# OPTML-Group/Unlearn-Saliency

Measured on AMD Instinct MI355X. Metric: unlearn_steps_per_sec (ResNet-18/CIFAR-10 10%-forget, RL + SalUn mask, batch 256/GPU), higher is better.
Workload: dtype f32

## Files before the change

### include/salun.h

```cpp
#ifndef SALUN_H
#define SALUN_H

#include <stddef.h>
#include <stdint.h>

#ifdef __cplusplus
extern "C" {
#endif

#define SALUN_OK 0
#define SALUN_EINVAL (-22)
#define SALUN_ENOSPC (-28)
#define SALUN_EIO (-5)

#define SALUN_MAX_THRESHOLDS 16

typedef void *salun_stream_t;

int salun_version(void);
const char *salun_strerror(int code);
const char *salun_arch(void);
int salun_clock_probe(unsigned long long *out , int samples, int spins, salun_stream_t stream);

int salun_saliency_accumulate(float *acc , const float *g ,
// ... 82 lines not shown
                               salun_stream_t stream);
int salun_conv2d_backward_data_add(const float *dy , const float *w , const float *addend ,
                                   float *dx , int N, int C, int H, int W, int K, int R, int stride, int pad,
                                   int P, int Q, salun_stream_t stream);
size_t salun_channel_sum_workspace_bytes(int N, int K);
int salun_channel_sum(const float *dy , float *out , int N, int K, int HW, int accumulate,
                      void *ws , size_t ws_bytes, salun_stream_t stream);
size_t salun_conv2d_wgrad_workspace_bytes(int N, int C, int K, int R, int P, int Q);
int salun_conv2d_backward_weight(const float *x , const float *dy , float *dw , int N, int C,
                                 int H, int W, int K, int R, int stride, int pad, int P, int Q, int accumulate,
                                 void *ws , size_t ws_bytes, salun_stream_t stream);
#define SALUN_WGRAD_SHARED 1u
int salun_conv2d_backward_weight_ex(const float *x , const float *dy , float *dw , int N, int C,
                                    int H, int W, int K, int R, int stride, int pad, int P, int Q, int accumulate,
                                    unsigned flags, void *ws , size_t ws_bytes, salun_stream_t stream);
#define SALUN_ROUTE_FORWARD 0
#define SALUN_ROUTE_BACKWARD_DATA 1
#define SALUN_ROUTE_BACKWARD_WEIGHT 2
#define SALUN_ROUTE_EPI 2u
#define SALUN_ROUTE_W_UNALIGNED 4u
#define SALUN_ROUTE_OUT_UNALIGNED 8u
#define SALUN_ROUTE_IN_UNALIGNED 16u
int salun_conv2d_route(int direction, int N, int C, int H, int W, int K, int R, int stride, int pad, int P, int Q,
                       unsigned flags, size_t ws_bytes, char *buf, size_t buflen, int *nsplit );

size_t salun_conv3x3_pack_bytes(int K, int C, int dgrad);
#define SALUN_PACK_MAX_JOBS 32
typedef struct {
  const float *w;
  float *img_fwd;
  float *img_dgrad;
  int32_t K, C;
} salun_pack_job_t;
int salun_conv3x3_pack_weights(const salun_pack_job_t *jobs , int njobs, salun_stream_t stream);
int salun_conv3x3_packed(const float *x , const float *img , const float *bias ,
                         const float *nbias , const float *addend , float *y ,
                         int N, int Cred, int H, int W, int Kout, int cfg, salun_stream_t stream);
// ... 300 lines not shown
```

### unlearn_saliency_amd/_lib.py

```python
from __future__ import annotations

import ctypes
import os
import subprocess

_HERE = os.path.dirname(os.path.abspath(__file__))
LIB_PATH = os.environ.get("SALUN_LIB") or os.path.join(_HERE, "libsalun.so")
CSRC_DIR = os.path.join(_HERE, "csrc")

SALUN_OK = 0
SALUN_EINVAL = -22
SALUN_ENOSPC = -28
SALUN_EIO = -5
SALUN_MAX_THRESHOLDS = 16
SALUN_TOPK_FORCE_FULL_SCAN = 1
SALUN_TOPK_VALUES_ONLY = 2
SALUN_WGRAD_SHARED = 1

c_void_p, c_int, c_int64, c_uint64 = ctypes.c_void_p, ctypes.c_int, ctypes.c_int64, ctypes.c_uint64
c_double, c_size_t = ctypes.c_double, ctypes.c_size_t

class GemmSeg(ctypes.Structure):
    _fields_ = [("A", c_void_p), ("B", c_void_p), ("K", ctypes.c_int32), ("a_i", ctypes.c_int32),
                ("a_k", ctypes.c_int32), ("b_j", ctypes.c_int32), ("b_k", ctypes.c_int32)]
# ... 75 lines not shown
    "salun_conv2d_forward": (c_int, [c_void_p, c_void_p, c_void_p, c_void_p] + [c_int] * 10 + [c_void_p]),
    "salun_conv2d_forward_fused": (c_int, [c_void_p] * 6 + [c_int] * 10 + [c_void_p, c_size_t, c_void_p]),
    "salun_conv2d_data_workspace_bytes": (c_size_t, [c_int] * 6),
    "salun_conv2d_backward_data_ws": (c_int, [c_void_p] * 4 + [c_int] * 10 + [c_void_p, c_size_t, c_void_p]),
    "salun_conv2d_backward_data": (c_int, [c_void_p, c_void_p, c_void_p] + [c_int] * 10 + [c_void_p]),
    "salun_channel_sum_workspace_bytes": (c_size_t, [c_int] * 2),
    "salun_channel_sum": (c_int, [c_void_p, c_void_p] + [c_int] * 4 + [c_void_p, c_size_t, c_void_p]),
    "salun_conv2d_wgrad_workspace_bytes": (c_size_t, [c_int] * 6),
    "salun_conv3x3_pack_bytes": (c_size_t, [c_int] * 3),
    "salun_conv3x3_pack_weights": (c_int, [c_void_p, c_int, c_void_p]),
    "salun_conv3x3_packed": (c_int, [c_void_p] * 6 + [c_int] * 6 + [c_void_p]),
    "salun_conv2d_backward_weight": (c_int, [c_void_p, c_void_p, c_void_p] + [c_int] * 11 + [c_void_p, c_size_t,
                                                                                          c_void_p]),
    "salun_conv2d_backward_weight_ex": (c_int, [c_void_p, c_void_p, c_void_p] + [c_int] * 11 + [ctypes.c_uint, c_void_p,
                                                                                                 c_size_t, c_void_p]),
    "salun_conv2d_route": (c_int, [c_int] * 11 + [ctypes.c_uint, c_size_t, ctypes.c_char_p, c_size_t,
                                   ctypes.POINTER(c_int)]),
    "salun_conv2d_bf16_supported": (c_int, [c_int] * 5),
    "salun_conv2d_bf16_pack_weights": (c_int, [c_void_p, c_void_p, c_int, c_int, c_int, c_void_p]),
    "salun_bf16_pack_weights_batch": (c_int, [c_void_p, c_int, c_void_p]),
    "salun_conv2d_bf16_data_workspace_bytes": (c_size_t, [c_int] * 8),
    "salun_conv2d_bf16_forward": (c_int, [c_void_p] * 6 + [c_int] * 8 + [c_void_p, c_size_t, c_void_p]),
    "salun_conv2d_bf16_backward_data": (c_int, [c_void_p] * 4 + [c_int] * 8 + [c_void_p, c_size_t, c_void_p]),
    "salun_conv2d_bf16_wgrad_workspace_bytes": (c_size_t, [c_int] * 8),
    "salun_conv2d_bf16_backward_weight": (c_int, [c_void_p] * 4 + [c_int] * 9 + [c_void_p, c_size_t, c_void_p]),
    "salun_colsum_bf16_workspace_bytes": (c_size_t, [c_int]),
    "salun_colsum_bf16": (c_int, [c_void_p, c_void_p, c_void_p, c_int64, c_int, c_int, c_int, c_void_p, c_size_t, c_void_p]),
    "salun_conv2d_bf16_backward_weight_ex": (c_int, [c_void_p] * 5 + [c_int] * 9 + [c_void_p, c_size_t, c_void_p]),
    "salun_conv2d_bf16_route": (c_int, [c_int] * 9 + [ctypes.c_uint, c_size_t, ctypes.c_char_p, c_size_t,
                                        ctypes.POINTER(c_int)]),
# ... 138 lines not shown
```

### unlearn_saliency_amd/csrc/salun_conv.hip

```cpp
#include "salun_common.h"
#include "salun_conv_plan.h"
#include <mutex>
#include <type_traits>
#include <unordered_set>

int salun_ring_wgrad_launch(const float *x, const float *dy, float *part, int N, int C, int H, int W, int K, int nsplit,
                            int nchunks, hipStream_t st);

namespace {

typedef float f32x16 __attribute__((ext_vector_type(16)));

struct PatchPos {
  int goff;
  int loff;
  int valid;
};

__device__ __forceinline__ void tile_origin(int tile, int NI, int TP, int tiles_per_img, int &n0, int &p0) {
  if (NI > 1) { n0 = tile * NI; p0 = 0; }
  else { n0 = tile / tiles_per_img; p0 = (tile - n0 * tiles_per_img) * TP; }
}

struct LanePix {
// ... 784 lines not shown
    }
  }
  float *out = part + (size_t)split * K * C * RS;
  const int c = c0 + ct * 32 + lo;
  if (c < C) {
#pragma unroll
    for (int t = 0; t < RS; ++t)
#pragma unroll
      for (int v = 0; v < 16; ++v) {
        const int k = k0 + kt * 32 + (v & 3) + 8 * (v >> 2) + 4 * hi;
        if (k < K) out[((size_t)t * K + k) * C + c] = acc[t][v];
      }
  }
}

template <int STRIDE, int NIT>
__global__ __launch_bounds__(256) void conv_wgrad_v(const float *__restrict__ x, const float *__restrict__ dy,
                                                    float *__restrict__ part, int N, int C, int H, int W, int K, int P,
                                                    int Q, int NI, int TP, int IH_t, int IW_t, int logQ, int nchunks) {
  constexpr int R = 3, RS = 9, PAD = 1;
  constexpr int PIXC = (STRIDE == 1) ? 64 : 32;
  constexpr int DROW = PIXC + 1;
  constexpr int NSTEP = PIXC / 2;
  constexpr int HALF = NSTEP / 2;
  constexpr int DN4 = 64 * PIXC / 4 / 256;
  constexpr int LOGPIX4 = (PIXC == 64) ? 4 : 3;
  constexpr int NLD = NIT + DN4;
  constexpr int LPS = (NLD + HALF - 1) / HALF;
  constexpr int NST = 4 * (NIT + DN4);
  constexpr int SPS = (NST + HALF - 1) / HALF;
  static_assert(LPS <= RS && SPS <= RS, "one staging instruction per MFMA slot at most");
  extern __shared__ __attribute__((aligned(16))) float lds[];
  const int PSZ = NI * IH_t * IW_t;
  const int ch_stride = PSZ | 1;
  const int BUF = 64 * ch_stride + 64 * DROW + 256;

  const int tid = threadIdx.x, lane = tid & 63, wave = tid >> 6;
  const int lo = lane & 31, hi = lane >> 5;
  const int kt = wave & 1, ct = wave >> 1;
  const int k0 = blockIdx.x * 64, c0 = blockIdx.y * 64;
  const int split = blockIdx.z, nsplit = gridDim.z;
  const int tiles_per_img = (NI > 1) ? 1 : P / TP;
  const int planeHW = H * W, PQ = P * Q;
  const int logTP = __builtin_ctz(TP);
  const int W4 = W >> 2;
  const int F4C = NI * IH_t * W4;

  f32x16 acc[RS];
#pragma unroll
  for (int t = 0; t < RS; ++t)
#pragma unroll
    for (int v = 0; v < 16; ++v) acc[t][v] = 0.f;

  int it_lds[NIT];
  int it_g[NIT];
  int it_ih[NIT], it_ni[NIT];
#pragma unroll
  for (int k = 0; k < NIT; ++k) {
    const int e = tid + k * 256;
    const int c = e / F4C, r = e - c * F4C;
    const int ni = r / (IH_t * W4), r2 = r - ni * (IH_t * W4);
    const int ih = r2 / W4, g4 = r2 - ih * W4;
    it_lds[k] = c * ch_stride + (ni * IH_t + ih) * IW_t + PAD + 4 * g4;
    it_g[k] = (ni * C + c) * planeHW + (ih - PAD) * W + 4 * g4;
    it_ih[k] = ih;
    it_ni[k] = ni;
  }
  float4 xreg[NIT];
  float4 dreg[DN4];
  const float *xbase = x;
  unsigned xoff[NIT], xmask[NIT];
  const float *dbase = dy;
  unsigned doff[DN4], dmask[DN4];
  int d_kk[DN4], d_ni[DN4], d_in[DN4];
#pragma unroll
  for (int i = 0; i < DN4; ++i) {
    const int e4 = tid + i * 256;
    const int kk = e4 >> LOGPIX4, m = (e4 & (PIXC / 4 - 1)) * 4;
    const int q = m & (Q - 1), pr = m >> logQ;
    d_kk[i] = kk;
    d_ni[i] = pr >> logTP;
    d_in[i] = (pr & (TP - 1)) * Q + q;
  }
  auto aim = [&](int chunk) {
    int n0, p0;
    if (NI > 1) { n0 = chunk * NI; p0 = 0; }
    else { n0 = chunk / tiles_per_img; p0 = (chunk - n0 * tiles_per_img) * TP; }
    xbase = x + ((size_t)n0 * C + c0) * planeHW;
    const int h0 = p0 * STRIDE;
#pragma unroll
    for (int k = 0; k < NIT; ++k) {
      const int h = h0 - PAD + it_ih[k];
      const bool ok = (n0 + it_ni[k]) < N && h >= 0 && h < H;
      xoff[k] = ok ? (unsigned)(it_g[k] + h0 * W) : 0u;
      xmask[k] = ok ? 0xffffffffu : 0u;
    }
    dbase = dy + ((size_t)n0 * K + k0) * PQ + (size_t)p0 * Q;
#pragma unroll
    for (int i = 0; i < DN4; ++i) {
      const bool okd = (n0 + d_ni[i]) < N && (k0 + d_kk[i]) < K;
      doff[i] = okd ? (unsigned)((d_ni[i] * K + d_kk[i]) * PQ + d_in[i]) : 0u;
      dmask[i] = okd ? 0xffffffffu : 0u;
    }
  };
  auto load_item = [&](int li) {
    if (li < NIT) xreg[li] = *reinterpret_cast<const float4 *>(xbase + xoff[li]);
    else dreg[li - NIT] = *reinterpret_cast<const float4 *>(dbase + doff[li - NIT]);
  };
  auto comp_of = [](const float4 &v, int comp) { return comp == 0 ? v.x : comp == 1 ? v.y : comp == 2 ? v.z : v.w; };
  auto store_item = [&](float *buf, int si) {
    if (si < 4 * NIT) {
      const int k = si >> 2, comp = si & 3;
      buf[it_lds[k] + comp] = __uint_as_float(__float_as_uint(comp_of(xreg[k], comp)) & xmask[k]);
    } else {
      const int sd = si - 4 * NIT, i = sd >> 2, comp = sd & 3;
      const int e4 = tid + i * 256;
      const int kk = e4 >> LOGPIX4, m = (e4 & (PIXC / 4 - 1)) * 4 + comp;
      (buf + 64 * ch_stride)[kk * DROW + m] = __uint_as_float(__float_as_uint(comp_of(dreg[i], comp)) & dmask[i]);
    }
  };

  for (int i = tid; i < 2 * BUF; i += 256) lds[i] = 0.f;
  __syncthreads();

  if (split < nchunks) {
    aim(split);
#pragma unroll
    for (int li = 0; li < NLD; ++li) load_item(li);
#pragma unroll
    for (int si = 0; si < NST; ++si) store_item(lds, si);
    __syncthreads();

    int cur = 0;
    for (int chunk = split; chunk < nchunks; chunk += nsplit) {
      const float *xp = lds + cur * BUF;
      const float *dl = xp + 64 * ch_stride;
      float *buf_n = lds + (cur ^ 1) * BUF;
      aim(chunk + nsplit < nchunks ? chunk + nsplit : chunk);
      const float *arow = dl + (kt * 32 + lo) * DROW + hi;
      const float *brow = xp + (ct * 32 + lo) * ch_stride + hi * STRIDE;
      auto pair_off = [&](int j) {
        const int q0 = j & (Q - 1), pr = j >> logQ;
        const int ni = pr >> logTP, pl = pr & (TP - 1);
        return (ni * IH_t + pl * STRIDE) * IW_t + q0 * STRIDE;
      };
      float a_cur, b_cur[RS], a_nxt = 0.f, b_nxt[RS];
      {
        const float *bp = brow + pair_off(0);
        a_cur = arow[0];
#pragma unroll
        for (int t = 0; t < RS; ++t) b_cur[t] = bp[(t / R) * IW_t + (t % R)];
      }
#pragma unroll
      for (int st = 0; st < NSTEP; ++st) {
        const float *bp = brow + ((st + 1 < NSTEP) ? pair_off(2 * st + 2) : 0);
#pragma unroll
        for (int t = 0; t < RS; ++t) {
          acc[t] = __builtin_amdgcn_mfma_f32_32x32x2f32(a_cur, b_cur[t], acc[t], 0, 0, 0);
          __builtin_amdgcn_sched_barrier(0);
          if (st + 1 < NSTEP) {
            if (t == 0) a_nxt = arow[2 * st + 2];
            b_nxt[t] = bp[(t / R) * IW_t + (t % R)];
          }
          if (st < HALF) {
            if (t < LPS && st * LPS + t < NLD) load_item(st * LPS + t);
          } else {
            if (t < SPS && (st - HALF) * SPS + t < NST) store_item(buf_n, (st - HALF) * SPS + t);
          }
          __builtin_amdgcn_sched_barrier(0);
        }
        a_cur = a_nxt;
#pragma unroll
        for (int t = 0; t < RS; ++t) b_cur[t] = b_nxt[t];
      }
      __syncthreads();
      cur ^= 1;
    }
  }
  float *out = part + (size_t)split * K * C * RS;
  const int c = c0 + ct * 32 + lo;
#pragma unroll
  for (int t = 0; t < RS; ++t)
#pragma unroll
    for (int v = 0; v < 16; ++v) {
      const int k = k0 + kt * 32 + (v & 3) + 8 * (v >> 2) + 4 * hi;
      if (k < K) out[((size_t)t * K + k) * C + c] = acc[t][v];
    }
}

template <int STRIDE>
__global__ __launch_bounds__(256) void conv_wgrad_1x1(const float *__restrict__ x, const float *__restrict__ dy,
                                                      float *__restrict__ part, int N, int C, int H, int W, int K,
                                                      int P, int Q, int nchunks) {
  constexpr int PIXC = 64, DROW = PIXC + 1, NSTEP = PIXC / 2, HALF = NSTEP / 2;
  constexpr int NA = 128 * PIXC / 4 / 256;
  constexpr int NB = NA;
  constexpr int NLD = NA + NB * STRIDE;
  constexpr int LPS = (NLD + HALF - 1) / HALF;
  constexpr int NST = 4 * (NA + NB);
  constexpr int SPS = (NST + HALF - 1) / HALF;
  static_assert(LPS <= 4 && SPS <= 4, "one staging instruction per MFMA slot");
  constexpr int BUF = 2 * 128 * DROW;
// ... 540 lines not shown
  int N, C, H, W, K, P, Q, pad;
};

template <int STRIDE>
void launch_one_wgrad_1x1(const WgradPlan &p, const WgradArgs &a, hipStream_t st) {
  allow_lds(conv_wgrad_1x1<STRIDE>, p.lds_bytes);
  hipLaunchKernelGGL(conv_wgrad_1x1<STRIDE>, dim3((a.K + 127) / 128, (a.C + 127) / 128, p.gz), dim3(256), p.lds_bytes, st,
                     a.x, a.dy, a.part, a.N, a.C, a.H, a.W, a.K, a.P, a.Q, p.nchunks);
}
template <int R, int STRIDE>
void launch_one_wgrad_smallc(const WgradPlan &p, const WgradArgs &a, hipStream_t st) {
  const TileGeom &g = p.g;
  hipLaunchKernelGGL((conv_wgrad_smallc<R, STRIDE>), dim3((a.K + 63) / 64, 1, p.gz), dim3(256), p.lds_bytes, st, a.x, a.dy,
                     a.part, a.N, a.C, a.H, a.W, a.K, a.P, a.Q, a.pad, g.NI, g.TP, g.IH_t, g.IW_t, g.logQ, g.ntiles);
}
template <int STRIDE, int NIT>
void launch_one_wgrad_v(const WgradPlan &p, const WgradArgs &a, hipStream_t st) {
  const TileGeom &g = p.g;
  allow_lds(conv_wgrad_v<STRIDE, NIT>, p.lds_bytes);
  hipLaunchKernelGGL((conv_wgrad_v<STRIDE, NIT>), dim3((a.K + 63) / 64, (a.C + 63) / 64, p.gz), dim3(256), p.lds_bytes, st,
                     a.x, a.dy, a.part, a.N, a.C, a.H, a.W, a.K, a.P, a.Q, g.NI, g.TP, g.IH_t, g.IW_t, g.logQ, g.ntiles);
}
template <int R, int STRIDE, bool FULLC>
void launch_one_wgrad(const WgradPlan &p, const WgradArgs &a, hipStream_t st) {
  const TileGeom &g = p.g;
  allow_lds(conv_wgrad<R, STRIDE, FULLC>, p.lds_bytes);
  hipLaunchKernelGGL((conv_wgrad<R, STRIDE, FULLC>), dim3((a.K + 63) / 64, (a.C + 63) / 64, p.gz), dim3(256), p.lds_bytes,
                     st, a.x, a.dy, a.part, a.N, a.C, a.H, a.W, a.K, a.P, a.Q, a.pad, g.NI, g.TP, g.IH_t, g.IW_t, g.logQ,
                     g.ntiles);
}

template <typename F>
inline void with_filter(int R, int stride, F &&f) {
  if (R == 3) { if (stride == 1) f(ic<3>{}, ic<1>{}); else f(ic<3>{}, ic<2>{}); }
  else { if (stride == 1) f(ic<1>{}, ic<1>{}); else f(ic<1>{}, ic<2>{}); }
}
// ... 17 lines not shown
        case 209: launch_one_wgrad_v<2, 9>(p, a, st); break;
        default: launch_one_wgrad_v<2, 10>(p, a, st); break;
      }
      break;
    case WG_GENERAL:
      with_filter(p.R, p.stride, [&](auto r, auto s) {
        if (p.fullC) launch_one_wgrad<decltype(r)::value, decltype(s)::value, true>(p, a, st);
        else launch_one_wgrad<decltype(r)::value, decltype(s)::value, false>(p, a, st);
      });
      break;
  }
  SALUN_LAUNCH_CHECK();
  return SALUN_OK;
}

}

SALUN_EXPORT size_t salun_conv2d_data_workspace_bytes(int N, int outC, int outH, int outW, int R, int conv_stride) {
  if (N < 1 || outC < 1 || outH < 1 || outW < 1 || (R != 1 && R != 3) || (conv_stride != 1 && conv_stride != 2)) return 0;
  const DataPlan p = plan_data(N, 1, outC, outH, outW, R, conv_stride, false, 1, false, false, false, 0);
  if (p.rc != SALUN_OK || p.wgs > 256 || (outH * outW) % 4 != 0) return 0;
  return (size_t)8 * N * outC * outH * outW * sizeof(float);
}

SALUN_EXPORT int salun_conv2d_forward_fused(const float *x, const float *w, const float *bias, const float *nbias,
                                            const float *addend, float *y, int N, int C, int H, int W, int K, int R,
                                            int stride, int pad, int P, int Q, void *ws, size_t ws_bytes,
                                            salun_stream_t stream) {
  if (!x || !w || !y || addend == y) return SALUN_EINVAL;
  const bool split_al16 = salun_aligned16(y) && salun_aligned16(ws) && (!addend || salun_aligned16(addend));
// ... 128 lines not shown
  return salun_conv2d_backward_weight_ex(x, dy, dw, N, C, H, W, K, R, stride, pad, P, Q, accumulate, 0, ws, ws_bytes, stream);
}

SALUN_EXPORT int salun_conv2d_backward_weight_ex(const float *x, const float *dy, float *dw, int N, int C, int H, int W,
                                                 int K, int R, int stride, int pad, int P, int Q, int accumulate,
                                                 unsigned flags, void *ws, size_t ws_bytes, salun_stream_t stream) {
  if (!x || !dy || !dw || !ws) return SALUN_EINVAL;
  const WgradPlan p = plan_wgrad(N, C, H, W, K, R, stride, pad, P, Q, (flags & SALUN_WGRAD_SHARED) != 0,
                                 salun_aligned16(x) && salun_aligned16(dy), ws_bytes);
  if (p.rc != SALUN_OK) return p.rc;
  hipStream_t st = salun_hip_stream(stream);
  const WgradArgs a{x, dy, static_cast<float *>(ws), N, C, H, W, K, P, Q, pad};
  const int rc = launch_wgrad(p, a, st);
  if (rc != SALUN_OK) return rc;
  launch_wgrad_reduce(a.part, dw, (int64_t)K * C * R * R, p.nsplit, accumulate, K * C, R * R, st);
  SALUN_LAUNCH_CHECK();
  return SALUN_OK;
}

SALUN_EXPORT int salun_conv2d_route(int direction, int N, int C, int H, int W, int K, int R, int stride, int pad, int P,
                                    int Q, unsigned flags, size_t ws_bytes, char *buf, size_t buflen, int *nsplit) {
  if (!buf || buflen < 1) return SALUN_EINVAL;
  buf[0] = 0;
  if (nsplit) *nsplit = 0;
  const bool w_al16 = !(flags & SALUN_ROUTE_W_UNALIGNED), out_al16 = !(flags & SALUN_ROUTE_OUT_UNALIGNED);
  const bool in_al16 = !(flags & SALUN_ROUTE_IN_UNALIGNED);
  int rc = SALUN_EINVAL, len = 0;
  if (direction == SALUN_ROUTE_FORWARD) {
    const DataPlan p = plan_data(N, C, K, P, Q, R, stride, false, C, (flags & SALUN_ROUTE_EPI) != 0, w_al16, out_al16,
                                 ws_bytes);
    if ((rc = p.rc) == SALUN_OK) len = data_label(buf, buflen, p);
  } else if (direction == SALUN_ROUTE_BACKWARD_DATA && (P < 1 || Q < 1)) {
  } else if (direction == SALUN_ROUTE_BACKWARD_DATA && stride == 1) {
    const DataPlan p = plan_data(N, K, C, H, W, R, 1, true, C, false, w_al16, out_al16, ws_bytes);
    if ((rc = p.rc) == SALUN_OK) len = data_label(buf, buflen, p);
  } else if (direction == SALUN_ROUTE_BACKWARD_DATA && stride == 2) {
    const Dgrad2Plan p = plan_dgrad_s2(N, C, H, W, K, R, pad, P, Q, w_al16, out_al16);
    if ((rc = p.rc) == SALUN_OK) len = dgrad2_label(buf, buflen, p);
  } else if (direction == SALUN_ROUTE_BACKWARD_WEIGHT) {
    const WgradPlan p = plan_wgrad(N, C, H, W, K, R, stride, pad, P, Q, (flags & SALUN_WGRAD_SHARED) != 0, in_al16,
                                   ws_bytes);
    if ((rc = p.rc) == SALUN_OK) {
      len = wgrad_label(buf, buflen, p);
      if (nsplit) *nsplit = p.nsplit;
    }
  }
  if (rc == SALUN_OK && (len < 0 || (size_t)len >= buflen)) { buf[0] = 0; return SALUN_ENOSPC; }
  return rc;
}
```

### unlearn_saliency_amd/csrc/salun_conv_plan.h

```cpp
#pragma once
#include <cstddef>
#include <cstdio>
#include "../../include/salun.h"

bool salun_ring_wgrad_fits(int N, int C, int H, int W, int K, int nchunks, bool in_al16);

namespace {

constexpr int CC = 8;
constexpr int igemm_chunk(int R, int stride) { return (R == 1 && stride == 1) ? 32 : CC; }

constexpr int tap_chunk(int taps) { return taps == 1 ? 32 : taps == 2 ? 16 : 8; }

struct TileGeom {
  int NI, TP, IH_t, IW_t, logQ;
  int ntiles;
  bool ok;
  int psz() const { return NI * IH_t * IW_t; }
};

inline int ilog2(int v) {
  int l = 0;
  while ((1 << l) < v) ++l;
  return l;
// ... 233 lines not shown

inline int wgrad_smallc_nsplit(int K, int nchunks) {
  int ns = 1024 / ((K + 63) / 64);
  if (ns > nchunks) ns = nchunks;
  return ns < 1 ? 1 : ns;
}
inline bool wgrad_is_smallc(int C, int R) { return C * R * R <= 32 && C <= 4; }

enum WgradRoute { WG_1X1, WG_SMALLC, WG_RING, WG_V, WG_GENERAL };
struct WgradPlan {
  int rc;
  WgradRoute route;
  int R, stride, W;
  bool fullC;
  int nit;
  int nchunks;
  int gz;
  int nsplit;
  size_t part_bytes;
  size_t lds_bytes;
  TileGeom g;
};

inline WgradPlan plan_wgrad(int N, int C, int H, int W, int K, int R, int stride, int pad, int P, int Q, bool shared,
                            bool in_al16 , size_t ws_bytes) {
  WgradPlan p{};
  p.rc = SALUN_EINVAL;
  p.R = R; p.stride = stride; p.W = W;
  if (N < 1 || C < 1 || K < 1 || P < 1 || Q < 1) return p;
  if (!((R == 3 || R == 1) && (stride == 1 || stride == 2))) return p;
// ... 40 lines not shown
    p.route = WG_RING;
    return p;
  }
  if (R == 3 && pad == 1 && p.fullC && W % 4 == 0 && Q * stride == W && P * stride == H && in_al16 &&
      (size_t)g.NI * C * H * W < (1u << 30)) {
    const int F4C = g.NI * g.IH_t * (W / 4);
    const int nit = (F4C % 4 == 0) ? F4C / 4 : 0;
    if (stride == 1 ? (nit == 5 || nit == 6 || nit == 8) : (nit == 9 || nit == 10)) {
      p.route = WG_V;
      p.nit = nit;
    }
  }
  return p;
}

inline int wgrad_label(char *buf, size_t n, const WgradPlan &p) {
  switch (p.route) {
    case WG_1X1: return snprintf(buf, n, "wgrad_1x1<%d>", p.stride);
    case WG_SMALLC: return snprintf(buf, n, "wgrad_smallc<%d,%d>", p.R, p.stride);
    case WG_RING: return snprintf(buf, n, "wgrad_ring<W%d>", p.W);
    case WG_V: return snprintf(buf, n, "wgrad_v<%d,%d>", p.stride, p.nit);
    default: return snprintf(buf, n, "wgrad<%d,%d,%s>", p.R, p.stride, p.fullC ? "true" : "false");
  }
}

}
```

### unlearn_saliency_amd/ops.py

```python
from __future__ import annotations

import ctypes
from typing import Optional, Sequence

import torch

from .fastfn import FastFunction

from . import _lib, ringpack, weightimg
from ._lib import c_double, c_int, c_int64, c_size_t, c_uint64, c_void_p, check
from .streams import _stream, _stream_handle


def _dev(t: Optional[torch.Tensor], dtype: torch.dtype, name: str, allow_none: bool = False) -> c_void_p:
    if t is None:
        if allow_none:
            return c_void_p(None)
        raise ValueError(f"{name} must not be None")
    if not t.is_cuda:
        raise RuntimeError(f"{name}: the SalUn HIP kernels need a device tensor (got {t.device}); no CPU fallback")
    if t.dtype != dtype:
        raise TypeError(f"{name}: expected {dtype}, got {t.dtype}")
    if not t.is_contiguous():
        raise ValueError(f"{name} must be contiguous")
# ... 402 lines not shown
    ws = workspace(nbytes, x.device, stream=stream)
    dw = out if out is not None else torch.empty(tuple(w_shape), dtype=torch.float32, device=x.device)
    rc = L.salun_conv2d_backward_weight_ex(_dev(x, torch.float32, "x"), _dev(dy, torch.float32, "dy"),
                                           _dev(dw, torch.float32, "dw"), N, C, H, W, K, R, stride, pad, P, Q,
                                           int(bool(accumulate and out is not None)),
                                           _lib.SALUN_WGRAD_SHARED if (shared if WGRAD_KERNEL[0] is None
                                                                       else WGRAD_KERNEL[0] == "shared") else 0,
                                           c_void_p(ws.data_ptr()), c_size_t(ws.numel()),
                                           c_void_p(_stream_handle() if stream is None else stream.cuda_stream))
    if rc == _lib.SALUN_EINVAL:
        return None
    check(rc, "salun_conv2d_backward_weight")
    return dw


def conv3x3_pack(w: torch.Tensor, dgrad: bool, out: Optional[torch.Tensor] = None) -> Optional[torch.Tensor]:
    K, C = w.shape[0], w.shape[1]
    L = _lib.lib()
    nbytes = int(L.salun_conv3x3_pack_bytes(K, C, int(dgrad)))
    if nbytes == 0 or tuple(w.shape[2:]) != (3, 3):
        return None
    img = out if out is not None and out.numel() * 4 == nbytes else torch.empty(nbytes // 4, dtype=torch.float32,
                                                                                device=w.device)
    _dev(w, torch.float32, "w")
    job = _lib.PackJob(w.data_ptr(), None if dgrad else img.data_ptr(), img.data_ptr() if dgrad else None, K, C)
    check(L.salun_conv3x3_pack_weights(ctypes.cast(ctypes.pointer(job), c_void_p), 1, _stream()),
          "salun_conv3x3_pack_weights")
    return img


# ... 561 lines not shown
```

### unlearn_saliency_amd/resblock.py

```python
from __future__ import annotations

import torch

from .fastfn import FastFunction
import torch.nn as nn

import os

from . import draws, gradsink, ops, wgrad_side

FWD_SHORTCUT_BESIDE = os.environ.get("SALUN_FWD_SHORTCUT_BESIDE", "1") != "0"


def _bn_args(bn: nn.BatchNorm2d):
    return bn.running_mean, bn.running_var, bn.training, bn.momentum, bn.eps


class _BasicBlockFn(FastFunction):
    @staticmethod
    def forward(ctx, x, blk, w1, g1, b1, w2, g2, b2, wd, gd, bd):
        s = blk.conv1.stride[0]
        N, C, H, W = x.shape
        P, Q = (H + 2 - 3) // s + 1, (W + 2 - 3) // s + 1
        training = blk.bn1.training
        cd = md = idd = None
        fork = None
# ... 11 lines not shown
                x.record_stream(fork)
        c1 = ops.conv2d_forward(x, w1, None, s, 1, P, Q)
        y1, m1, i1 = ops.bn_forward(c1, None, g1, b1, *_bn_args(blk.bn1), True, blk.bn1.num_batches_tracked)
        c2 = ops.conv2d_forward(y1, w2, None, 1, 1, P, Q)
        if wd is None:
            skip = x
        elif fork is None:
            cd, skip, md, idd = shortcut()
        else:
            main.wait_stream(fork)
            for t in (cd, skip, md, idd):
                if t is not None:
                    t.record_stream(main)
        out, m2, i2 = ops.bn_forward(c2, skip, g2, b2, *_bn_args(blk.bn2), True, blk.bn2.num_batches_tracked)
        ctx.save_for_backward(x, c1, y1, c2, out, cd, w1, g1, b1, w2, g2, b2, wd, gd, bd, m1, i1, m2, i2, md, idd)
        ctx.cfg = (s, training)
        return out

    @staticmethod
    def backward(ctx, dout):
        x, c1, y1, c2, out, cd, w1, g1, b1, w2, g2, b2, wd, gd, bd, m1, i1, m2, i2, md, idd = ctx.saved_tensors
        s, training = ctx.cfg
        dout = dout.contiguous()
        grads = {}

        def bn_bwd(dy, y, xin, g, b, m, i, relu, want_dres):
            to_g, to_b = gradsink.pair(g, b)
            dx, dres, dg, db = ops.bn_backward(dy, y, xin, g, m, i, training, relu, want_dres, to_g.out, to_b.out)
            return dx, dres, to_g.returned(dg), to_b.returned(db)

        wgrad = wgrad_side.ConvWgrad(dout.device)

        dc2, dskip, dg2, db2 = bn_bwd(dout, out, c2, g2, b2, m2, i2, True, True)
        dwd = dgd = dbd = None
        dxd = dskip
        if wd is not None:
            dcd, _, dgd, dbd = bn_bwd(dskip, None, cd, gd, bd, md, idd, False, False)
            dwd = wgrad(x, dcd, wd, s, 0)
            dxd = ops.conv2d_backward_data(dcd, wd, x.shape, s, 0) if ctx.needs_input_grad[0] else None
        dw2 = wgrad(y1, dc2, w2, 1, 1)
        dy1 = ops.conv2d_backward_data(dc2, w2, y1.shape, 1, 1)
        dc1, _, dg1, db1 = bn_bwd(dy1, y1, c1, g1, b1, m1, i1, True, False)
        dw1 = wgrad(x, dc1, w1, s, 1)
        dx = ops.conv2d_backward_data(dc1, w1, x.shape, s, 1, addend=dxd) if ctx.needs_input_grad[0] else None
        wgrad.finish()
        return dx, None, dw1, dg1, db1, dw2, dg2, db2, dwd, dgd, dbd


def _probe(blk, shape, device) -> bool:
    N, C, H, W = shape
    s = blk.conv1.stride[0]
    P, Q = (H + 2 - 3) // s + 1, (W + 2 - 3) // s + 1
    K = blk.conv1.out_channels
    if (P * Q) % 4 or (H * W) % 4:
        return False
    e = lambda *sh: torch.empty(sh, dtype=torch.float32, device=device)
    x, y1, dy = e(N, C, H, W), e(N, K, P, Q), e(N, K, P, Q)
    convs = [(x, blk.conv1.weight, s, 1), (y1, blk.conv2.weight, 1, 1)]
    if blk.downsample is not None:
        convs.append((x, blk.downsample[0].weight, s, 0))
    for xin, w, st, pad in convs:
        if ops.conv2d_forward(xin, w, None, st, pad, P, Q) is None:
            return False
        if ops.conv2d_backward_data(dy, w, xin.shape, st, pad, addend=xin) is None:
            return False
        if ops.conv2d_backward_weight(xin, dy, w.shape, st, pad) is None:
            return False
    return True


def _structure_ok(blk) -> bool:
    convs = [blk.conv1, blk.conv2] + ([blk.downsample[0]] if blk.downsample is not None else [])
    bns = [blk.bn1, blk.bn2] + ([blk.downsample[1]] if blk.downsample is not None else [])
    if any(type(b) is not nn.BatchNorm2d or not b.affine or not b.track_running_stats or b.momentum is None
           for b in bns):
        return False
    if any(c.bias is not None or c.groups != 1 or c.dilation != (1, 1) or c.weight.dtype != torch.float32
           for c in convs):
        return False
    if len({b.training for b in bns}) != 1:
        return False
    c1, c2 = blk.conv1, blk.conv2
# ... 165 lines not shown
```

### unlearn_saliency_amd/wgrad_side.py

```python
from __future__ import annotations

import os
from typing import Optional

import torch

from . import gradsink, ops, streams

OVERLAP = os.environ.get("SALUN_WGRAD_OVERLAP", "1") != "0"


class overlap_disabled:

    def __enter__(self):
        global OVERLAP
        self._prev = OVERLAP
        OVERLAP = False
        return self

    def __exit__(self, *exc):
        global OVERLAP
        OVERLAP = self._prev
        return False

# ... 50 lines not shown


def reset_join_state() -> None:
    _join_queued.clear()
    _held.clear()
    for dev, side in _streams.items():
        torch.cuda.current_stream(dev).wait_stream(side)


def beside(device: torch.device, reads, launch, alloc: bool = False):
    main, side = torch.cuda.current_stream(device), stream(device)
    side.wait_stream(main)
    if alloc:
        with torch.cuda.stream(side):
            out = launch(side)
        if out is not None:
            out.record_stream(main)
    else:
        out = launch(side)
    if out is not None:
        for t in reads:
            t.record_stream(side)
        hold_until_join(reads[-1])
        _join_at_end_of_backward(device)
    return out


class ConvWgrad:
    __slots__ = ("device", "overlap", "join")

    def __init__(self, device: torch.device):
        self.device, self.overlap, self.join = device, OVERLAP, False

    def __call__(self, xin, dy, w, stride: int, pad: int):
        d = gradsink.dest(w)
        if self.overlap:
            dw = beside(self.device, (xin, dy), lambda side: ops.conv2d_backward_weight(
                xin, dy, w.shape, stride, pad, out=d.out, accumulate=d.accumulate, shared=True, stream=side),
                alloc=not d.accumulate)
        else:
            dw = ops.conv2d_backward_weight(xin, dy, w.shape, stride, pad, out=d.out, accumulate=d.accumulate)
        dw = d.returned(dw)
        if dw is not None:
            self.join = self.overlap
        return dw

    def finish(self) -> None:
        if self.join:
            torch.cuda.current_stream(self.device).wait_stream(stream(self.device))
            release_held(self.device)
```

Before: 117.9.

## Fuse downsample 1x1 projection wgrad into stride-2 3x3 conv1 wgrad kernel

For ResNet blocks with a stride-2 downsample, the 1x1 projection weight gradient is computed inside the 3x3 conv1 weight-gradient kernel. It reuses the centre tap of the shared input patch, staging the projection's output gradient as a second LDS tile and adding a tenth MFMA per step. This saves a separate pass over the input activation and one kernel launch, at the cost of more LDS, more registers and a wider workspace. A probe at shape-check time decides per block whether the fused path is allowed, and the old separate launches remain as the fallback.

```diff
diff --git a/include/salun.h b/include/salun.h
--- a/include/salun.h
+++ b/include/salun.h
@@ -120,6 +120,11 @@
 int salun_conv2d_backward_weight_ex(const float *x , const float *dy , float *dw , int N, int C,
                                     int H, int W, int K, int R, int stride, int pad, int P, int Q, int accumulate,
                                     unsigned flags, void *ws , size_t ws_bytes, salun_stream_t stream);
+size_t salun_conv2d_wgrad_proj_workspace_bytes(int N, int C, int H, int W, int K, int P, int Q);
+int salun_conv2d_backward_weight_proj(const float *x , const float *dy , const float *dyp ,
+                                      float *dw , float *dwp , int N, int C, int H, int W, int K, int P,
+                                      int Q, int accumulate, int accumulate_p, unsigned flags, void *ws ,
+                                      size_t ws_bytes, salun_stream_t stream);
 #define SALUN_ROUTE_FORWARD 0
 #define SALUN_ROUTE_BACKWARD_DATA 1
 #define SALUN_ROUTE_BACKWARD_WEIGHT 2
@@ -127,6 +132,7 @@
 #define SALUN_ROUTE_W_UNALIGNED 4u
 #define SALUN_ROUTE_OUT_UNALIGNED 8u
 #define SALUN_ROUTE_IN_UNALIGNED 16u
+#define SALUN_ROUTE_WGRAD_PROJ 32u
 int salun_conv2d_route(int direction, int N, int C, int H, int W, int K, int R, int stride, int pad, int P, int Q,
                        unsigned flags, size_t ws_bytes, char *buf, size_t buflen, int *nsplit );
 
diff --git a/unlearn_saliency_amd/_lib.py b/unlearn_saliency_amd/_lib.py
--- a/unlearn_saliency_amd/_lib.py
+++ b/unlearn_saliency_amd/_lib.py
@@ -113,6 +113,9 @@
                                                                                           c_void_p]),
     "salun_conv2d_backward_weight_ex": (c_int, [c_void_p, c_void_p, c_void_p] + [c_int] * 11 + [ctypes.c_uint, c_void_p,
                                                                                                  c_size_t, c_void_p]),
+    "salun_conv2d_wgrad_proj_workspace_bytes": (c_size_t, [c_int] * 7),
+    "salun_conv2d_backward_weight_proj": (c_int, [c_void_p] * 5 + [c_int] * 9 + [ctypes.c_uint, c_void_p, c_size_t,
+                                                                                c_void_p]),
     "salun_conv2d_route": (c_int, [c_int] * 11 + [ctypes.c_uint, c_size_t, ctypes.c_char_p, c_size_t,
                                    ctypes.POINTER(c_int)]),
     "salun_conv2d_bf16_supported": (c_int, [c_int] * 5),
diff --git a/unlearn_saliency_amd/csrc/salun_conv.hip b/unlearn_saliency_amd/csrc/salun_conv.hip
--- a/unlearn_saliency_amd/csrc/salun_conv.hip
+++ b/unlearn_saliency_amd/csrc/salun_conv.hip
@@ -822,10 +822,12 @@
   }
 }
 
-template <int STRIDE, int NIT>
+template <int STRIDE, int NIT, bool PROJ = false>
 __global__ __launch_bounds__(256) void conv_wgrad_v(const float *__restrict__ x, const float *__restrict__ dy,
                                                     float *__restrict__ part, int N, int C, int H, int W, int K, int P,
-                                                    int Q, int NI, int TP, int IH_t, int IW_t, int logQ, int nchunks) {
+                                                    int Q, int NI, int TP, int IH_t, int IW_t, int logQ, int nchunks,
+                                                    const float *__restrict__ dyp) {
+  static_assert(!PROJ || STRIDE == 2, "the projection shares the centre tap of a stride-2 patch");
   constexpr int R = 3, RS = 9, PAD = 1;
   constexpr int PIXC = (STRIDE == 1) ? 64 : 32;
   constexpr int DROW = PIXC + 1;
@@ -833,15 +835,18 @@
   constexpr int HALF = NSTEP / 2;
   constexpr int DN4 = 64 * PIXC / 4 / 256;
   constexpr int LOGPIX4 = (PIXC == 64) ? 4 : 3;
-  constexpr int NLD = NIT + DN4;
+  constexpr int ND = PROJ ? 2 * DN4 : DN4;
+  constexpr int NTILE = PROJ ? 2 : 1;
+  constexpr int NSLOT = PROJ ? RS + 1 : RS;
+  constexpr int NLD = NIT + ND;
   constexpr int LPS = (NLD + HALF - 1) / HALF;
-  constexpr int NST = 4 * (NIT + DN4);
+  constexpr int NST = 4 * (NIT + ND);
   constexpr int SPS = (NST + HALF - 1) / HALF;
-  static_assert(LPS <= RS && SPS <= RS, "one staging instruction per MFMA slot at most");
+  static_assert(LPS <= NSLOT && SPS <= NSLOT, "one staging instruction per MFMA slot at most");
   extern __shared__ __attribute__((aligned(16))) float lds[];
   const int PSZ = NI * IH_t * IW_t;
   const int ch_stride = PSZ | 1;
-  const int BUF = 64 * ch_stride + 64 * DROW + 256;
+  const int BUF = 64 * ch_stride + NTILE * 64 * DROW + 256;
 
   const int tid = threadIdx.x, lane = tid & 63, wave = tid >> 6;
   const int lo = lane & 31, hi = lane >> 5;
@@ -859,6 +864,9 @@
   for (int t = 0; t < RS; ++t)
 #pragma unroll
     for (int v = 0; v < 16; ++v) acc[t][v] = 0.f;
+  f32x16 acc_p;
+#pragma unroll
+  for (int v = 0; v < 16; ++v) acc_p[v] = 0.f;
 
   int it_lds[NIT];
   int it_g[NIT];
@@ -875,10 +883,10 @@
     it_ni[k] = ni;
   }
   float4 xreg[NIT];
-  float4 dreg[DN4];
+  float4 dreg[ND];
   const float *xbase = x;
   unsigned xoff[NIT], xmask[NIT];
-  const float *dbase = dy;
+  const float *dbase = dy, *dpbase = dyp;
   unsigned doff[DN4], dmask[DN4];
   int d_kk[DN4], d_ni[DN4], d_in[DN4];
 #pragma unroll
@@ -904,6 +912,7 @@
       xmask[k] = ok ? 0xffffffffu : 0u;
     }
     dbase = dy + ((size_t)n0 * K + k0) * PQ + (size_t)p0 * Q;
+    if constexpr (PROJ) dpbase = dyp + ((size_t)n0 * K + k0) * PQ + (size_t)p0 * Q;
 #pragma unroll
     for (int i = 0; i < DN4; ++i) {
       const bool okd = (n0 + d_ni[i]) < N && (k0 + d_kk[i]) < K;
@@ -913,7 +922,8 @@
   };
   auto load_item = [&](int li) {
     if (li < NIT) xreg[li] = *reinterpret_cast<const float4 *>(xbase + xoff[li]);
-    else dreg[li - NIT] = *reinterpret_cast<const float4 *>(dbase + doff[li - NIT]);
+    else if (li < NIT + DN4) dreg[li - NIT] = *reinterpret_cast<const float4 *>(dbase + doff[li - NIT]);
+    else dreg[li - NIT] = *reinterpret_cast<const float4 *>(dpbase + doff[li - NIT - DN4]);
   };
   auto comp_of = [](const float4 &v, int comp) { return comp == 0 ? v.x : comp == 1 ? v.y : comp == 2 ? v.z : v.w; };
   auto store_item = [&](float *buf, int si) {
@@ -921,10 +931,12 @@
       const int k = si >> 2, comp = si & 3;
       buf[it_lds[k] + comp] = __uint_as_float(__float_as_uint(comp_of(xreg[k], comp)) & xmask[k]);
     } else {
-      const int sd = si - 4 * NIT, i = sd >> 2, comp = sd & 3;
+      const int sd = si - 4 * NIT, j = sd >> 2, comp = sd & 3;
+      const int i = j % DN4, tile = j / DN4;
       const int e4 = tid + i * 256;
       const int kk = e4 >> LOGPIX4, m = (e4 & (PIXC / 4 - 1)) * 4 + comp;
-      (buf + 64 * ch_stride)[kk * DROW + m] = __uint_as_float(__float_as_uint(comp_of(dreg[i], comp)) & dmask[i]);
+      (buf + 64 * ch_stride + tile * 64 * DROW)[kk * DROW + m] =
+          __uint_as_float(__float_as_uint(comp_of(dreg[j], comp)) & dmask[i]);
     }
   };
 
@@ -953,9 +965,12 @@
         return (ni * IH_t + pl * STRIDE) * IW_t + q0 * STRIDE;
       };
       float a_cur, b_cur[RS], a_nxt = 0.f, b_nxt[RS];
+      const float *arow_p = arow + 64 * DROW;
+      float ap_cur = 0.f, ap_nxt = 0.f;
       {
         const float *bp = brow + pair_off(0);
         a_cur = arow[0];
+        if constexpr (PROJ) ap_cur = arow_p[0];
 #pragma unroll
         for (int t = 0; t < RS; ++t) b_cur[t] = bp[(t / R) * IW_t + (t % R)];
       }
@@ -963,12 +978,14 @@
       for (int st = 0; st < NSTEP; ++st) {
         const float *bp = brow + ((st + 1 < NSTEP) ? pair_off(2 * st + 2) : 0);
 #pragma unroll
-        for (int t = 0; t < RS; ++t) {
-          acc[t] = __builtin_amdgcn_mfma_f32_32x32x2f32(a_cur, b_cur[t], acc[t], 0, 0, 0);
+        for (int t = 0; t < NSLOT; ++t) {
+          if (t < RS) acc[t] = __builtin_amdgcn_mfma_f32_32x32x2f32(a_cur, b_cur[t], acc[t], 0, 0, 0);
+          else acc_p = __builtin_amdgcn_mfma_f32_32x32x2f32(ap_cur, b_cur[4], acc_p, 0, 0, 0);
           __builtin_amdgcn_sched_barrier(0);
           if (st + 1 < NSTEP) {
             if (t == 0) a_nxt = arow[2 * st + 2];
-            b_nxt[t] = bp[(t / R) * IW_t + (t % R)];
+            if (t < RS) b_nxt[t] = bp[(t / R) * IW_t + (t % R)];
+            else ap_nxt = arow_p[2 * st + 2];
           }
           if (st < HALF) {
             if (t < LPS && st * LPS + t < NLD) load_item(st * LPS + t);
@@ -978,6 +995,7 @@
           __builtin_amdgcn_sched_barrier(0);
         }
         a_cur = a_nxt;
+        ap_cur = ap_nxt;
 #pragma unroll
         for (int t = 0; t < RS; ++t) b_cur[t] = b_nxt[t];
       }
@@ -994,6 +1012,14 @@
       const int k = k0 + kt * 32 + (v & 3) + 8 * (v >> 2) + 4 * hi;
       if (k < K) out[((size_t)t * K + k) * C + c] = acc[t][v];
     }
+  if constexpr (PROJ) {
+    float *outp = part + ((size_t)nsplit * RS + split) * K * C;
+#pragma unroll
+    for (int v = 0; v < 16; ++v) {
+      const int k = k0 + kt * 32 + (v & 3) + 8 * (v >> 2) + 4 * hi;
+      if (k < K) outp[(size_t)k * C + c] = acc_p[v];
+    }
+  }
 }
 
 template <int STRIDE>
@@ -1564,12 +1590,13 @@
   hipLaunchKernelGGL((conv_wgrad_smallc<R, STRIDE>), dim3((a.K + 63) / 64, 1, p.gz), dim3(256), p.lds_bytes, st, a.x, a.dy,
                      a.part, a.N, a.C, a.H, a.W, a.K, a.P, a.Q, a.pad, g.NI, g.TP, g.IH_t, g.IW_t, g.logQ, g.ntiles);
 }
-template <int STRIDE, int NIT>
-void launch_one_wgrad_v(const WgradPlan &p, const WgradArgs &a, hipStream_t st) {
+template <int STRIDE, int NIT, bool PROJ = false>
+void launch_one_wgrad_v(const WgradPlan &p, const WgradArgs &a, hipStream_t st, const float *dyp = nullptr) {
   const TileGeom &g = p.g;
-  allow_lds(conv_wgrad_v<STRIDE, NIT>, p.lds_bytes);
-  hipLaunchKernelGGL((conv_wgrad_v<STRIDE, NIT>), dim3((a.K + 63) / 64, (a.C + 63) / 64, p.gz), dim3(256), p.lds_bytes, st,
-                     a.x, a.dy, a.part, a.N, a.C, a.H, a.W, a.K, a.P, a.Q, g.NI, g.TP, g.IH_t, g.IW_t, g.logQ, g.ntiles);
+  allow_lds(conv_wgrad_v<STRIDE, NIT, PROJ>, p.lds_bytes);
+  hipLaunchKernelGGL((conv_wgrad_v<STRIDE, NIT, PROJ>), dim3((a.K + 63) / 64, (a.C + 63) / 64, p.gz), dim3(256),
+                     p.lds_bytes, st, a.x, a.dy, a.part, a.N, a.C, a.H, a.W, a.K, a.P, a.Q, g.NI, g.TP, g.IH_t, g.IW_t,
+                     g.logQ, g.ntiles, dyp);
 }
 template <int R, int STRIDE, bool FULLC>
 void launch_one_wgrad(const WgradPlan &p, const WgradArgs &a, hipStream_t st) {
@@ -1617,6 +1644,13 @@
   return SALUN_OK;
 }
 
+inline int launch_wgrad_proj(const WgradPlan &p, const WgradArgs &a, const float *dyp, hipStream_t st) {
+  if (p.nit == 9) launch_one_wgrad_v<2, 9, true>(p, a, st, dyp);
+  else launch_one_wgrad_v<2, 10, true>(p, a, st, dyp);
+  SALUN_LAUNCH_CHECK();
+  return SALUN_OK;
+}
+
 }
 
 SALUN_EXPORT size_t salun_conv2d_data_workspace_bytes(int N, int outC, int outH, int outW, int R, int conv_stride) {
@@ -1775,6 +1809,31 @@
   const int rc = launch_wgrad(p, a, st);
   if (rc != SALUN_OK) return rc;
   launch_wgrad_reduce(a.part, dw, (int64_t)K * C * R * R, p.nsplit, accumulate, K * C, R * R, st);
+  SALUN_LAUNCH_CHECK();
+  return SALUN_OK;
+}
+
+SALUN_EXPORT size_t salun_conv2d_wgrad_proj_workspace_bytes(int N, int C, int H, int W, int K, int P, int Q) {
+  const WgradPlan p = plan_wgrad_proj(N, C, H, W, K, P, Q, true, true, ~(size_t)0);
+  return p.rc == SALUN_OK ? p.part_bytes : 0;
+}
+
+SALUN_EXPORT int salun_conv2d_backward_weight_proj(const float *x, const float *dy, const float *dyp, float *dw,
+                                                   float *dwp, int N, int C, int H, int W, int K, int P, int Q,
+                                                   int accumulate, int accumulate_p, unsigned flags, void *ws,
+                                                   size_t ws_bytes, salun_stream_t stream) {
+  if (!x || !dy || !dyp || !dw || !dwp || !ws) return SALUN_EINVAL;
+  const WgradPlan p = plan_wgrad_proj(N, C, H, W, K, P, Q, (flags & SALUN_WGRAD_SHARED) != 0,
+                                      salun_aligned16(x) && salun_aligned16(dy) && salun_aligned16(dyp), ws_bytes);
+  if (p.rc != SALUN_OK) return p.rc;
+  hipStream_t st = salun_hip_stream(stream);
+  const WgradArgs a{x, dy, static_cast<float *>(ws), N, C, H, W, K, P, Q, 1};
+  const int rc = launch_wgrad_proj(p, a, dyp, st);
+  if (rc != SALUN_OK) return rc;
+  const int64_t KC = (int64_t)K * C;
+  launch_wgrad_reduce(a.part, dw, KC * 9, p.nsplit, accumulate, K * C, 9, st);
+  SALUN_LAUNCH_CHECK();
+  launch_wgrad_reduce(a.part + (size_t)p.nsplit * 9 * KC, dwp, KC, p.nsplit, accumulate_p, K * C, 1, st);
   SALUN_LAUNCH_CHECK();
   return SALUN_OK;
 }
@@ -1798,6 +1857,14 @@
   } else if (direction == SALUN_ROUTE_BACKWARD_DATA && stride == 2) {
     const Dgrad2Plan p = plan_dgrad_s2(N, C, H, W, K, R, pad, P, Q, w_al16, out_al16);
     if ((rc = p.rc) == SALUN_OK) len = dgrad2_label(buf, buflen, p);
+  } else if (direction == SALUN_ROUTE_BACKWARD_WEIGHT && (flags & SALUN_ROUTE_WGRAD_PROJ)) {
+    if (R == 3 && stride == 2 && pad == 1) {
+      const WgradPlan p = plan_wgrad_proj(N, C, H, W, K, P, Q, (flags & SALUN_WGRAD_SHARED) != 0, in_al16, ws_bytes);
+      if ((rc = p.rc) == SALUN_OK) {
+        len = wgrad_label(buf, buflen, p);
+        if (nsplit) *nsplit = p.nsplit;
+      }
+    }
   } else if (direction == SALUN_ROUTE_BACKWARD_WEIGHT) {
     const WgradPlan p = plan_wgrad(N, C, H, W, K, R, stride, pad, P, Q, (flags & SALUN_WGRAD_SHARED) != 0, in_al16,
                                    ws_bytes);
diff --git a/unlearn_saliency_amd/csrc/salun_conv_plan.h b/unlearn_saliency_amd/csrc/salun_conv_plan.h
--- a/unlearn_saliency_amd/csrc/salun_conv_plan.h
+++ b/unlearn_saliency_amd/csrc/salun_conv_plan.h
@@ -271,6 +271,7 @@
   int R, stride, W;
   bool fullC;
   int nit;
+  bool proj;
   int nchunks;
   int gz;
   int nsplit;
@@ -341,12 +342,26 @@
   return p;
 }
 
+inline WgradPlan plan_wgrad_proj(int N, int C, int H, int W, int K, int P, int Q, bool shared,
+                                 bool in_al16 , size_t ws_bytes) {
+  WgradPlan p = plan_wgrad(N, C, H, W, K, 3, 2, 1, P, Q, shared, in_al16, ~(size_t)0);
+  if (p.rc != SALUN_OK) return p;
+  p.rc = SALUN_EINVAL;
+  if (p.route != WG_V || p.stride != 2) return p;
+  p.lds_bytes += sizeof(float) * 2 * 64 * 33;
+  if (p.lds_bytes > 160 * 1024) return p;
+  p.proj = true;
+  p.part_bytes = sizeof(float) * (size_t)p.nsplit * K * C * 10;
+  p.rc = ws_bytes < p.part_bytes ? SALUN_ENOSPC : SALUN_OK;
+  return p;
+}
+
 inline int wgrad_label(char *buf, size_t n, const WgradPlan &p) {
   switch (p.route) {
     case WG_1X1: return snprintf(buf, n, "wgrad_1x1<%d>", p.stride);
     case WG_SMALLC: return snprintf(buf, n, "wgrad_smallc<%d,%d>", p.R, p.stride);
     case WG_RING: return snprintf(buf, n, "wgrad_ring<W%d>", p.W);
-    case WG_V: return snprintf(buf, n, "wgrad_v<%d,%d>", p.stride, p.nit);
+    case WG_V: return snprintf(buf, n, "wgrad_v<%d,%d>%s", p.stride, p.nit, p.proj ? "+proj" : "");
     default: return snprintf(buf, n, "wgrad<%d,%d,%s>", p.R, p.stride, p.fullC ? "true" : "false");
   }
 }
diff --git a/unlearn_saliency_amd/ops.py b/unlearn_saliency_amd/ops.py
--- a/unlearn_saliency_amd/ops.py
+++ b/unlearn_saliency_amd/ops.py
@@ -440,6 +440,36 @@
     return dw
 
 
+def conv2d_backward_weight_proj(x: torch.Tensor, dy: torch.Tensor, dyp: torch.Tensor, w_shape, wp_shape,
+                                out: Optional[torch.Tensor] = None, accumulate: bool = False,
+                                out_p: Optional[torch.Tensor] = None, accumulate_p: bool = False,
+                                shared: bool = False, stream: Optional[torch.cuda.Stream] = None):
+    N, C, H, W = x.shape
+    K, P, Q = dy.shape[1], dy.shape[2], dy.shape[3]
+    if (tuple(w_shape) != (K, C, 3, 3) or tuple(wp_shape) != (K, C, 1, 1) or dyp.shape != dy.shape
+            or not dyp.is_contiguous()):
+        return None
+    L = _lib.lib()
+    nbytes = L.salun_conv2d_wgrad_proj_workspace_bytes(N, C, H, W, K, P, Q)
+    if nbytes == 0:
+        return None
+    ws = workspace(nbytes, x.device, stream=stream)
+    dw = out if out is not None else torch.empty(tuple(w_shape), dtype=torch.float32, device=x.device)
+    dwp = out_p if out_p is not None else torch.empty(tuple(wp_shape), dtype=torch.float32, device=x.device)
+    rc = L.salun_conv2d_backward_weight_proj(_dev(x, torch.float32, "x"), _dev(dy, torch.float32, "dy"),
+                                             _dev(dyp, torch.float32, "dyp"), _dev(dw, torch.float32, "dw"),
+                                             _dev(dwp, torch.float32, "dwp"), N, C, H, W, K, P, Q,
+                                             int(bool(accumulate and out is not None)),
+                                             int(bool(accumulate_p and out_p is not None)),
+                                             _lib.SALUN_WGRAD_SHARED if shared else 0,
+                                             c_void_p(ws.data_ptr()), c_size_t(ws.numel()),
+                                             c_void_p(_stream_handle() if stream is None else stream.cuda_stream))
+    if rc == _lib.SALUN_EINVAL:
+        return None
+    check(rc, "salun_conv2d_backward_weight_proj")
+    return dw, dwp
+
+
 def conv3x3_pack(w: torch.Tensor, dgrad: bool, out: Optional[torch.Tensor] = None) -> Optional[torch.Tensor]:
     K, C = w.shape[0], w.shape[1]
     L = _lib.lib()
diff --git a/unlearn_saliency_amd/resblock.py b/unlearn_saliency_amd/resblock.py
--- a/unlearn_saliency_amd/resblock.py
+++ b/unlearn_saliency_amd/resblock.py
@@ -10,6 +10,7 @@
 from . import draws, gradsink, ops, wgrad_side
 
 FWD_SHORTCUT_BESIDE = os.environ.get("SALUN_FWD_SHORTCUT_BESIDE", "1") != "0"
+WGRAD_PROJ_FUSED = True
 
 
 def _bn_args(bn: nn.BatchNorm2d):
@@ -51,13 +52,14 @@
                     t.record_stream(main)
         out, m2, i2 = ops.bn_forward(c2, skip, g2, b2, *_bn_args(blk.bn2), True, blk.bn2.num_batches_tracked)
         ctx.save_for_backward(x, c1, y1, c2, out, cd, w1, g1, b1, w2, g2, b2, wd, gd, bd, m1, i1, m2, i2, md, idd)
-        ctx.cfg = (s, training)
+        pair_ok = wd is not None and blk.__dict__.get("_wgrad_proj_shapes", {}).get((tuple(x.shape), x.device), False)
+        ctx.cfg = (s, training, pair_ok)
         return out
 
     @staticmethod
     def backward(ctx, dout):
         x, c1, y1, c2, out, cd, w1, g1, b1, w2, g2, b2, wd, gd, bd, m1, i1, m2, i2, md, idd = ctx.saved_tensors
-        s, training = ctx.cfg
+        s, training, pair_ok = ctx.cfg
         dout = dout.contiguous()
         grads = {}
 
@@ -68,17 +70,25 @@
 
         wgrad = wgrad_side.ConvWgrad(dout.device)
 
+        fuse = pair_ok and WGRAD_PROJ_FUSED
         dc2, dskip, dg2, db2 = bn_bwd(dout, out, c2, g2, b2, m2, i2, True, True)
-        dwd = dgd = dbd = None
+        dwd = dgd = dbd = dcd = None
         dxd = dskip
         if wd is not None:
             dcd, _, dgd, dbd = bn_bwd(dskip, None, cd, gd, bd, md, idd, False, False)
-            dwd = wgrad(x, dcd, wd, s, 0)
-            dxd = ops.conv2d_backward_data(dcd, wd, x.shape, s, 0) if ctx.needs_input_grad[0] else None
+            if not fuse:
+                dwd = wgrad(x, dcd, wd, s, 0)
+            dxd =ops.conv2d_backward_data(dcd, wd, x.shape, s, 0) if ctx.needs_input_grad[0] else None
         dw2 = wgrad(y1, dc2, w2, 1, 1)
         dy1 = ops.conv2d_backward_data(dc2, w2, y1.shape, 1, 1)
         dc1, _, dg1, db1 = bn_bwd(dy1, y1, c1, g1, b1, m1, i1, True, False)
-        dw1 = wgrad(x, dc1, w1, s, 1)
+        both = wgrad.pair(x, dc1, w1, dcd, wd) if fuse else None
+        if both is not None:
+            dw1, dwd = both
+        else:
+            if fuse:
+                dwd = wgrad(x, dcd, wd, s, 0)
+            dw1 = wgrad(x, dc1, w1, s, 1)
         dx = ops.conv2d_backward_data(dc1, w1, x.shape, s, 1, addend=dxd) if ctx.needs_input_grad[0] else None
         wgrad.finish()
         return dx, None, dw1, dg1, db1, dw2, dg2, db2, dwd, dgd, dbd
@@ -103,6 +113,9 @@
             return False
         if ops.conv2d_backward_weight(xin, dy, w.shape, st, pad) is None:
             return False
+    if blk.downsample is not None:
+        pair = ops.conv2d_backward_weight_proj(x, dy, dy, blk.conv1.weight.shape, blk.downsample[0].weight.shape)
+        blk.__dict__.setdefault("_wgrad_proj_shapes", {})[(tuple(shape), device)] = pair is not None
     return True
 
 
diff --git a/unlearn_saliency_amd/wgrad_side.py b/unlearn_saliency_amd/wgrad_side.py
--- a/unlearn_saliency_amd/wgrad_side.py
+++ b/unlearn_saliency_amd/wgrad_side.py
@@ -88,8 +88,9 @@
     if alloc:
         with torch.cuda.stream(side):
             out = launch(side)
-        if out is not None:
-            out.record_stream(main)
+        for t in (out if isinstance(out, tuple) else (out,)):
+            if t is not None:
+                t.record_stream(main)
     else:
         out = launch(side)
     if out is not None:
@@ -119,6 +120,23 @@
             self.join = self.overlap
         return dw
 
+    def pair(self, xin, dy, w, dyp, wp):
+        d, dp = gradsink.dest(w), gradsink.dest(wp)
+        launch = lambda shared, side: ops.conv2d_backward_weight_proj(
+            xin, dy, dyp, w.shape, wp.shape, out=d.out, accumulate=d.accumulate, out_p=dp.out,
+            accumulate_p=dp.accumulate, shared=shared, stream=side)
+        if self.overlap:
+            res = beside(self.device, (xin, dyp, dy), lambda side: launch(True, side),
+                         alloc=not (d.accumulate and dp.accumulate))
+        else:
+            res = launch(False, None)
+        if res is None:
+            return None
+        dw, dwp = d.returned(res[0]), dp.returned(res[1])
+        if dw is not None or dwp is not None:
+            self.join = self.overlap
+        return dw, dwp
+
     def finish(self) -> None:
         if self.join:
             torch.cuda.current_stream(self.device).wait_stream(stream(self.device))
```

New measurement: 118.7 (median of 6 runs). No clear change (+0.6%).
